# pratyushkumar211/industrial_nnmpc_2021

Measured on AMD Instinct MI355X. Metric: condensed-QP solves/sec (CDU offline datagen), higher is better.
Workload: dtype f64; 1 GPU; cdu_offline_data: synthetic CDU-size plant (n=4480 vars, m=8960 box rows, n_aug=284), 100000 sampled x0 per GPU per step, whole sequences u* written out; batch_per_gpu=100000, total_batch=100000, method=auto, parallelism=dp1 (sharded samples, 1 RCCL gather of the first moves pe...

## Files before the change

industrial_nnmpc_2021_amd/csrc/qp_predict.h:

```cpp
#pragma once
#include "qp_asm.h"

namespace nnmpc {

typedef __bf16 pbf16x8 __attribute__((ext_vector_type(8)));
typedef float pf32x4 __attribute__((ext_vector_type(4)));
typedef unsigned int pu32x4 __attribute__((ext_vector_type(4)));
typedef unsigned int pu32x2 __attribute__((ext_vector_type(2)));
typedef float pf32x2 __attribute__((ext_vector_type(2)));
typedef __bf16 pbf16x2 __attribute__((ext_vector_type(2)));
typedef _Float16 pf16x2 __attribute__((ext_vector_type(2)));

constexpr int PRED_NW = 8;
constexpr int PRED_MAXIT = 64;
template <int NT> struct PredCfg {
  static constexpr int W = 16 * NT * PRED_NW;
  static constexpr int KS = W / 32;
  static constexpr int LDY = W + 8;
};
constexpr int PRED_W = PredCfg<4>::W;
constexpr int PRED_W2 = PredCfg<8>::W;

struct PredArgs {
  const pu32x4* Hf;
  int iters;
  int* itsum;
  int fac10;
  int adaptive;
  float beta[PRED_MAXIT];
};

template <int NT, int PT> __host__ __device__ constexpr int pred_lds_bytes(int nu) {
  return 16 * PT * PredCfg<NT>::LDY * 2 + 2 * 16 * PT * (nu + 4) * 4 + 16;
}

template <int NT> __host__ __device__ constexpr size_t pred_frag_index(int jtg, int ks, int lane) {
  return (((size_t)(jtg / NT) * PredCfg<NT>::KS + ks) * NT + (jtg % NT)) * 64 + lane;
}

__device__ __forceinline__ unsigned pred_bf16(float x) {
  const unsigned u = __float_as_uint(x);
  return (u + 0x7fffu + ((u >> 16) & 1u)) >> 16;
}

template <int NT, int PT, bool NU4 = true>
__global__ __launch_bounds__(64 * PRED_NW, 2) void asm_predict_k(AsmDev d, PredArgs a) {
  extern __shared__ __attribute__((aligned(16))) unsigned char sm_raw[];
  constexpr int KS = PredCfg<NT>::KS, LDY = PredCfg<NT>::LDY, MR = 16 * PT;
  unsigned short* Y = reinterpret_cast<unsigned short*>(sm_raw);
  const int ldb = d.nu + 4;
  float* lbs = reinterpret_cast<float*>(Y + MR * LDY);
  float* ubs = lbs + MR * ldb;
  int* nviol = reinterpret_cast<int*>(ubs + MR * ldb);
  float* rsum = reinterpret_cast<float*>(nviol + 1);
  constexpr int NTH = 64 * PRED_NW;
  const int tid = threadIdx.x, lane = tid & 63, w = __builtin_amdgcn_readfirstlane(tid >> 6);
  const int li = lane & 15, lq = lane >> 4;
  const int p0 = blockIdx.x * MR;
  for (int i = tid; i < MR * d.nu; i += NTH) {
    const int r = i / d.nu, k = i - r * d.nu;
    const size_t p = (size_t)min(p0 + r, d.nseg - 1);
    lbs[r * ldb + k] = (float)d.lb[p * d.nu + k];
    ubs[r * ldb + k] = (float)d.ub[p * d.nu + k];
  }
  for (int i = tid; i < MR * LDY / 2; i += NTH) reinterpret_cast<unsigned*>(Y)[i] = 0u;
  if (tid == 0) { *nviol = 0; rsum[0] = 0.f; rsum[1] = 0.f; }
  unsigned sx[NT][PT][2], sm[NT][PT][2];
#pragma unroll
  for (int jt = 0; jt < NT; ++jt)
#pragma unroll
    for (int pt = 0; pt < PT; ++pt) {
      const size_t p = (size_t)min(p0 + 16 * pt + li, d.nseg - 1);
      const double* xr = d.xunc + p * d.np + 16 * (w * NT + jt) + 4 * lq;
#pragma unroll
      for (int h = 0; h < 2; ++h) {
        const pf32x2 xu = {fminf(fmaxf((float)xr[2 * h], -60000.f), 60000.f), fminf(fmaxf((float)xr[2 * h + 1], -60000.f), 60000.f)};
        sx[jt][pt][h] = __builtin_bit_cast(unsigned, __builtin_convertvector(xu, pf16x2));
        sm[jt][pt][h] = 0u;
      }
    }
  int kc0[NT];
#pragma unroll
  for (int jt = 0; jt < NT; ++jt) kc0[jt] = (16 * (w * NT + jt) + 4 * lq) % d.nu;
  const bool st_words = (d.n & 3) == 0;
  const bool per32 = 32 % d.nu == 0;
  __syncthreads();
  const __amdgpu_buffer_rsrc_t rH = __builtin_amdgcn_make_buffer_rsrc(const_cast<pu32x4*>(a.Hf), 0, PRED_NW * KS * NT * 1024, 0x00020000);
  const int l16 = lane * 16;
  const int hw0 = w * (KS * NT * 1024);
  auto hload = [&](int ksn, int jt) __attribute__((always_inline)) {
    return __builtin_bit_cast(pu32x4, __builtin_amdgcn_raw_buffer_load_b128(rH, l16 + jt * 1024, hw0 + ksn * (NT * 1024), 0));
  };
  int nit = a.iters;
  int kb = 0;
  for (int it = 0; it < nit; ++it) {
    if (tid == 0) rsum[it & 1] = 0.f;
    pf32x4 acc[NT][PT];
#pragma unroll
    for (int jt = 0; jt < NT; ++jt)
#pragma unroll
      for (int pt = 0; pt < PT; ++pt) acc[jt][pt] = pf32x4{0.f, 0.f, 0.f, 0.f};
#ifdef PRED_NO_MFMA
    if (false) {
#else
    if (it > 0) {
#endif
      constexpr int RD = 3;
      pu32x4 hb[RD][NT];
      asm_sfor<0, RD - 1>([&](auto bc) __attribute__((always_inline)) {
        constexpr int b = decltype(bc)::value;
#pragma unroll
        for (int jt = 0; jt < NT; ++jt) hb[b][jt] = hload(b, jt);
      });
      asm_sfor<0, KS>([&](auto kc) __attribute__((always_inline)) {
        constexpr int ks = decltype(kc)::value, b = ks % RD;
        if constexpr (ks + RD - 1 < KS) {
#pragma unroll
          for (int jt = 0; jt < NT; ++jt) hb[(ks + RD - 1) % RD][jt] = hload(ks + RD - 1, jt);
        }
        pu32x4 yf[PT];
#pragma unroll
        for (int pt = 0; pt < PT; ++pt) yf[pt] = *reinterpret_cast<const pu32x4*>(Y + (16 * pt + li) * LDY + 32 * ks + 8 * lq);
#pragma unroll
        for (int jt = 0; jt < NT; ++jt)
#pragma unroll
          for (int pt = 0; pt < PT; ++pt)
            acc[jt][pt] = __builtin_amdgcn_mfma_f32_16x16x32_bf16(__builtin_bit_cast(pbf16x8, hb[b][jt]), __builtin_bit_cast(pbf16x8, yf[pt]),
                                                                  acc[jt][pt], 0, 0, 0);
        __builtin_amdgcn_sched_barrier(0);
      });
    }
    __syncthreads();
    if (it > 0) kb = rsum[(it - 1) & 1] > 0.f ? 0 : kb + 1;
    const pf32x2 beta2 = {a.beta[kb], a.beta[kb]};
    pf32x2 rdot = {0.f, 0.f};
    int yo = li * LDY + 16 * NT * w + 4 * lq, bo = li * ldb;
    asm volatile("" : "+v"(yo), "+v"(bo));
    unsigned short* Yl = Y + yo;
    const float* lbl = lbs + bo;
    const float* ubl = ubs + bo;
    int nv0 = 0;
#pragma unroll
    for (int pt = 0; pt < PT; ++pt) {
      pf32x4 lb4[2], ub4[2];
#pragma unroll
      for (int jt = 0; jt < NT; ++jt) {
        if constexpr (NU4) {
          if (jt < 2 || !per32) {
            lb4[jt & 1] = *reinterpret_cast<const pf32x4*>(lbl + 16 * pt * ldb + kc0[jt]);
            ub4[jt & 1] = *reinterpret_cast<const pf32x4*>(ubl + 16 * pt * ldb + kc0[jt]);
          }
        } else {
#pragma unroll
          for (int r = 0; r < 4; ++r) {
            const int k = kc0[jt] + r, kk = k >= d.nu ? k - d.nu : k;
            lb4[jt & 1][r] = lbl[16 * pt * ldb + kk];
            ub4[jt & 1][r] = ubl[16 * pt * ldb + kk];
          }
        }
        unsigned short* yp = Yl + 16 * pt * LDY + 16 * jt;
        const pu32x2 yw = *reinterpret_cast<const pu32x2*>(yp);
        unsigned yb[2];
#pragma unroll
        for (int h = 0; h < 2; ++h) {
          const pf32x2 xu = __builtin_convertvector(__builtin_bit_cast(pf16x2, sx[jt][pt][h]), pf32x2);
          const unsigned mw = sm[jt][pt][h], ywd = yw[h];
          const pf32x2 nu = {__uint_as_float(mw << 16), __uint_as_float(mw & 0xffff0000u)};
          const pf32x2 y = {__uint_as_float(ywd << 16), __uint_as_float(ywd & 0xffff0000u)};
          const pf32x2 ac = {acc[jt][pt][2 * h], acc[jt][pt][2 * h + 1]};
#ifdef PRED_NO_EPI
          const pf32x2 wv = xu - ac;
#else
          const pf32x2 wv = y + (xu - ac);
#endif
          const pf32x2 cl = {__builtin_amdgcn_fmed3f(wv[0], lb4[jt & 1][2 * h], ub4[jt & 1][2 * h]),
                             __builtin_amdgcn_fmed3f(wv[1], lb4[jt & 1][2 * h + 1], ub4[jt & 1][2 * h + 1])};
          const pf32x2 nun = wv - cl;
          const pf32x2 dn = nun - nu;
          const pf32x2 yn = beta2 * dn + nun;
          rdot += (y - nun) * dn;
          yb[h] = __builtin_bit_cast(unsigned, __builtin_convertvector(yn, pbf16x2));
          sm[jt][pt][h] = __builtin_bit_cast(unsigned, __builtin_convertvector(nun, pbf16x2));
        }
        *reinterpret_cast<pu32x2*>(yp) = pu32x2{yb[0], yb[1]};
      }
      __builtin_amdgcn_sched_barrier(0);
    }
    {
      float rd = rdot[0] + rdot[1];
      for (int off = 32; off > 0; off >>= 1) rd += __shfl_xor(rd, off);
      if (lane == 0) atomicAdd(&rsum[it & 1], rd);
    }
    if (it == 0 && a.adaptive) {
#pragma unroll
      for (int jt = 0; jt < NT; ++jt)
#pragma unroll
        for (int pt = 0; pt < PT; ++pt)
#pragma unroll
          for (int h = 0; h < 2; ++h) nv0 += ((sm[jt][pt][h] & 0x7fffu) != 0u) + ((sm[jt][pt][h] & 0x7fff0000u) != 0u);
      for (int off = 32; off > 0; off >>= 1) nv0 += __shfl_xor(nv0, off);
      if (lane == 0 && nv0) atomicAdd(nviol, nv0);
    }
    __syncthreads();
    if (it == 0 && a.adaptive) nit = min(a.iters, max(8, (a.fac10 * *nviol) / (10 * MR)));
    if (it == 0 && tid == 0 && a.itsum) atomicAdd(a.itsum, nit - 1);
  }
#pragma unroll
  for (int jt = 0; jt < NT; ++jt) {
    const int c0 = 16 * (w * NT + jt) + 4 * lq;
#pragma unroll
    for (int pt = 0; pt < PT; ++pt) {
      const int p = p0 + 16 * pt + li;
      unsigned wd = 0;
#pragma unroll
      for (int r = 0; r < 4; ++r) {
        const unsigned hb16 = (sm[jt][pt][r >> 1] >> (16 * (r & 1))) & 0xffffu;
        wd |= ((hb16 & 0x7fffu) == 0u ? 0u : ((hb16 >> 15) ? 2u : 1u)) << (8 * r);
      }
      if (p < d.nseg && st_words && c0 + 3 < d.n) *reinterpret_cast<unsigned*>(d.st + (size_t)p * d.n + c0) = wd;
      else if (p < d.nseg) {
#pragma unroll
        for (int r = 0; r < 4; ++r) if (c0 + r < d.n) d.st[(size_t)p * d.n + c0 + r] = (unsigned char)((wd >> (8 * r)) & 0xff);
      }
    }
  }
}

__global__ __launch_bounds__(256) void asm_extent_k(AsmDev d, int c0, int c1, int* cnt) {
  __shared__ int wsum[4];
  const int lane = threadIdx.x & 63, wave = threadIdx.x >> 6;
  int hit = 0;
  for (int q = 0; q < 16; ++q) {
    const int p = blockIdx.x * 64 + wave * 16 + q;
    if (p >= d.nseg) break;
    int v = 0;
    for (int r = c0 + lane; r < c1; r += 64) {
      const int k = r % d.nu;
      const double x = d.xunc[(size_t)p * d.np + r];
      v |= x > d.ub[(size_t)p * d.nu + k] || x < d.lb[(size_t)p * d.nu + k];
    }
    hit += __any(v) ? 1 : 0;
  }
  if (lane == 0) wsum[wave] = hit;
  __syncthreads();
  if (threadIdx.x == 0) { const int t = wsum[0] + wsum[1] + wsum[2] + wsum[3]; if (t) atomicAdd(cnt, t); }
}

}
```

Measured before the change: 8.198 million solves/s.

## Overlap prox epilogue of one column half with MFMA k-steps of the other

Splits each wave's column tiles into two halves across the matrix and reorders the Hessian fragment layout so the K loop runs in quarters. While one half's matvec runs on the MFMA units, the projection and momentum epilogue of the other half is interleaved into the same k-steps, hiding the VALU work behind matrix ops. To free registers, half of the unconstrained-solution values move from registers to LDS. The cost is a more complex software pipeline, extra LDS use, and a changed Y read order that depends on the Y halves being updated in the right sequence.

```diff
diff --git a/industrial_nnmpc_2021_amd/csrc/qp_predict.h b/industrial_nnmpc_2021_amd/csrc/qp_predict.h
--- a/industrial_nnmpc_2021_amd/csrc/qp_predict.h
+++ b/industrial_nnmpc_2021_amd/csrc/qp_predict.h
@@ -31,11 +31,17 @@
 };
 
 template <int NT, int PT> __host__ __device__ constexpr int pred_lds_bytes(int nu) {
-  return 16 * PT * PredCfg<NT>::LDY * 2 + 2 * 16 * PT * (nu + 4) * 4 + 16;
+  return 16 * PT * PredCfg<NT>::LDY * 2 + 2 * 16 * PT * (nu + 4) * 4 + 16 + 16 * PT * PredCfg<NT>::W;
+}
+
+template <int NT> __host__ __device__ constexpr int pred_col_tile(int w, int jt) {
+  return (jt / (NT / 2)) * (PRED_NW * (NT / 2)) + w * (NT / 2) + jt % (NT / 2);
 }
 
 template <int NT> __host__ __device__ constexpr size_t pred_frag_index(int jtg, int ks, int lane) {
-  return (((size_t)(jtg / NT) * PredCfg<NT>::KS + ks) * NT + (jtg % NT)) * 64 + lane;
+  constexpr int NH = NT / 2, KQ = PredCfg<NT>::KS / 2;
+  const int c = jtg / (PRED_NW * NH), w = (jtg / NH) % PRED_NW, j = jtg % NH, h = ks / KQ, kl = ks % KQ;
+  return (((((size_t)w * 2 + h) * 2 + c) * KQ + kl) * NH + j) * 64 + lane;
 }
 
 __device__ __forceinline__ unsigned pred_bf16(float x) {
@@ -53,6 +59,7 @@
   float* ubs = lbs + MR * ldb;
   int* nviol = reinterpret_cast<int*>(ubs + MR * ldb);
   float* rsum = reinterpret_cast<float*>(nviol + 1);
+  pu32x2* xul = reinterpret_cast<pu32x2*>(nviol + 4);
   constexpr int NTH = 64 * PRED_NW;
   const int tid = threadIdx.x, lane = tid & 63, w = __builtin_amdgcn_readfirstlane(tid >> 6);
   const int li = lane & 15, lq = lane >> 4;
@@ -65,149 +72,216 @@
   }
   for (int i = tid; i < MR * LDY / 2; i += NTH) reinterpret_cast<unsigned*>(Y)[i] = 0u;
   if (tid == 0) { *nviol = 0; rsum[0] = 0.f; rsum[1] = 0.f; }
-  unsigned sx[NT][PT][2], sm[NT][PT][2];
+  static_assert(NT % 2 == 0 && (PT == 2 || PT == 4), "the schedule below: NT / 2 tiles per half, 4 / PT k-steps per tile of the prox");
+  constexpr int NH = NT / 2;
+  unsigned sx[NH][PT][2], sm[NT][PT][2];
 #pragma unroll
   for (int jt = 0; jt < NT; ++jt)
 #pragma unroll
     for (int pt = 0; pt < PT; ++pt) {
+      unsigned xp[2];
       const size_t p = (size_t)min(p0 + 16 * pt + li, d.nseg - 1);
-      const double* xr = d.xunc + p * d.np + 16 * (w * NT + jt) + 4 * lq;
+      const double* xr = d.xunc + p * d.np + 16 * pred_col_tile<NT>(w, jt) + 4 * lq;
 #pragma unroll
       for (int h = 0; h < 2; ++h) {
         const pf32x2 xu = {fminf(fmaxf((float)xr[2 * h], -60000.f), 60000.f), fminf(fmaxf((float)xr[2 * h + 1], -60000.f), 60000.f)};
-        sx[jt][pt][h] = __builtin_bit_cast(unsigned, __builtin_convertvector(xu, pf16x2));
+        xp[h] = __builtin_bit_cast(unsigned, __builtin_convertvector(xu, pf16x2));
         sm[jt][pt][h] = 0u;
       }
+      if (jt < NH) { sx[jt % NH][pt][0] = xp[0]; sx[jt % NH][pt][1] = xp[1]; }
+      else xul[((jt - NH) * PT + pt) * NTH + tid] = pu32x2{xp[0], xp[1]};
     }
   int kc0[NT];
 #pragma unroll
-  for (int jt = 0; jt < NT; ++jt) kc0[jt] = (16 * (w * NT + jt) + 4 * lq) % d.nu;
+  for (int jt = 0; jt < NT; ++jt) kc0[jt] = (16 * pred_col_tile<NT>(w, jt) + 4 * lq) % d.nu;
   const bool st_words = (d.n & 3) == 0;
-  const bool per32 = 32 % d.nu == 0;
   __syncthreads();
   const __amdgpu_buffer_rsrc_t rH = __builtin_amdgcn_make_buffer_rsrc(const_cast<pu32x4*>(a.Hf), 0, PRED_NW * KS * NT * 1024, 0x00020000);
   const int l16 = lane * 16;
   const int hw0 = w * (KS * NT * 1024);
-  auto hload = [&](int ksn, int jt) __attribute__((always_inline)) {
-    return __builtin_bit_cast(pu32x4, __builtin_amdgcn_raw_buffer_load_b128(rH, l16 + jt * 1024, hw0 + ksn * (NT * 1024), 0));
+  constexpr int KQ = KS / 2, NS = 4 * KQ;
+  constexpr int RD = 3;
+  constexpr int KPU = 4 / PT;
+  auto hload = [&](int s, int j) __attribute__((always_inline)) {
+    return __builtin_bit_cast(pu32x4, __builtin_amdgcn_raw_buffer_load_b128(rH, l16 + j * 1024, hw0 + s * (NH * 1024), 0));
+  };
+  pu32x4 hb[RD][NH];
+  pu32x4 yf[2][PT];
+  pf32x4 acc[NT][PT];
+  pf32x2 rdot = {0.f, 0.f};
+  pf32x2 beta2 = {a.beta[0], a.beta[0]};
+  int yo, bo, xo;
+  auto launder = [&]() __attribute__((always_inline)) {
+    yo = li * LDY + 16 * NH * w + 4 * lq; bo = li * ldb; xo = tid;
+    asm volatile("" : "+v"(yo), "+v"(bo), "+v"(xo));
+  };
+  auto etile = [&](auto jtc, auto ptc) __attribute__((always_inline)) {
+    constexpr int jt = decltype(jtc)::value, pt = decltype(ptc)::value;
+    const float* lbl = lbs + bo + 16 * pt * ldb;
+    const float* ubl = ubs + bo + 16 * pt * ldb;
+    pf32x4 lb4, ub4;
+    if constexpr (NU4) {
+      lb4 = *reinterpret_cast<const pf32x4*>(lbl + kc0[jt]);
+      ub4 = *reinterpret_cast<const pf32x4*>(ubl + kc0[jt]);
+    } else {
+#pragma unroll
+      for (int r = 0; r < 4; ++r) {
+        const int k = kc0[jt] + r, kk = k >= d.nu ? k - d.nu : k;
+        lb4[r] = lbl[kk];
+        ub4[r] = ubl[kk];
+      }
+    }
+    unsigned short* yp = Y + yo + 16 * pt * LDY + (jt / NH) * (PredCfg<NT>::W / 2) + 16 * (jt % NH);
+    const pu32x2 yw = *reinterpret_cast<const pu32x2*>(yp);
+    unsigned yb[2];
+    unsigned xp[2];
+    if constexpr (jt < NH) {
+      asm volatile("" : "+v"(sx[jt][pt][0]), "+v"(sx[jt][pt][1]));
+      xp[0] = sx[jt][pt][0]; xp[1] = sx[jt][pt][1];
+    } else {
+      const pu32x2 xw = xul[xo + ((jt - NH) * PT + pt) * NTH];
+      xp[0] = xw[0]; xp[1] = xw[1];
+    }
+#pragma unroll
+    for (int h = 0; h < 2; ++h) {
+      const pf32x2 xu = __builtin_convertvector(__builtin_bit_cast(pf16x2, xp[h]), pf32x2);
+      const unsigned mw = sm[jt][pt][h], ywd = yw[h];
+      const pf32x2 nu = {__uint_as_float(mw << 16), __uint_as_float(mw & 0xffff0000u)};
+      const pf32x2 y = {__uint_as_float(ywd << 16), __uint_as_float(ywd & 0xffff0000u)};
+      const pf32x2 ac = {acc[jt][pt][2 * h], acc[jt][pt][2 * h + 1]};
+#ifdef PRED_NO_EPI
+      const pf32x2 wv = xu - ac;
+#else
+      const pf32x2 wv = y + (xu - ac);
+#endif
+      const pf32x2 cl = {__builtin_amdgcn_fmed3f(wv[0], lb4[2 * h], ub4[2 * h]), __builtin_amdgcn_fmed3f(wv[1], lb4[2 * h + 1], ub4[2 * h + 1])};
+      const pf32x2 nun = wv - cl;
+      const pf32x2 dn = nun - nu;
+      const pf32x2 yn = beta2 * dn + nun;
+      rdot += (y - nun) * dn;
+      yb[h] = __builtin_bit_cast(unsigned, __builtin_convertvector(yn, pbf16x2));
+      sm[jt][pt][h] = __builtin_bit_cast(unsigned, __builtin_convertvector(nun, pbf16x2));
+    }
+    *reinterpret_cast<pu32x2*>(yp) = pu32x2{yb[0], yb[1]};
+  };
+  auto ehalf = [&](auto cc) __attribute__((always_inline)) {
+    constexpr int c = decltype(cc)::value;
+    asm_sfor<0, PT>([&](auto ptc) __attribute__((always_inline)) {
+      asm_sfor<0, NH>([&](auto jc) __attribute__((always_inline)) { etile(asm_ic<c * NH + decltype(jc)::value>{}, ptc); });
+      __builtin_amdgcn_sched_barrier(0);
+    });
+  };
+  auto rflush = [&](int slot) __attribute__((always_inline)) {
+    float rd = rdot[0] + rdot[1];
+    for (int off = 32; off > 0; off >>= 1) rd += __shfl_xor(rd, off);
+    if (lane == 0) atomicAdd(&rsum[slot], rd);
+    rdot = pf32x2{0.f, 0.f};
+  };
+  auto kstep = [&](auto sc) __attribute__((always_inline)) {
+#ifndef PRED_NO_MFMA
+    constexpr int s = decltype(sc)::value, c = (s / KQ) & 1, sn = s + RD - 1;
+    if constexpr (sn < NS) {
+#pragma unroll
+      for (int j = 0; j < NH; ++j) hb[sn % RD][j] = hload(sn, j);
+    }
+    auto yread = [&](auto tc) __attribute__((always_inline)) {
+      constexpr int t = decltype(tc)::value, ks = (t / (2 * KQ)) * KQ + t % KQ;
+#pragma unroll
+      for (int pt = 0; pt < PT; ++pt) yf[t & 1][pt] = *reinterpret_cast<const pu32x4*>(Y + (16 * pt + li) * LDY + 32 * ks + 8 * lq);
+    };
+    if constexpr (s % (2 * KQ) == 0) yread(asm_ic<s>{});
+    if constexpr ((s + 1) % (2 * KQ) != 0) yread(asm_ic<s + 1>{});
+#pragma unroll
+    for (int j = 0; j < NH; ++j)
+#pragma unroll
+      for (int pt = 0; pt < PT; ++pt)
+        acc[c * NH + j][pt] = __builtin_amdgcn_mfma_f32_16x16x32_bf16(__builtin_bit_cast(pbf16x8, hb[s % RD][j]), __builtin_bit_cast(pbf16x8, yf[s & 1][pt]),
+                                                                      acc[c * NH + j][pt], 0, 0, 0);
+#endif
+  };
+  auto ringfill = [&]() __attribute__((always_inline)) {
+#ifndef PRED_NO_MFMA
+    asm_sfor<0, RD - 1>([&](auto bc) __attribute__((always_inline)) {
+      constexpr int b = decltype(bc)::value;
+#pragma unroll
+      for (int j = 0; j < NH; ++j) hb[b][j] = hload(b, j);
+    });
+#endif
+  };
+  auto quarter = [&](auto qc, auto ec) __attribute__((always_inline)) {
+    constexpr int q = decltype(qc)::value, c = q & 1;
+    constexpr bool WITH_E = decltype(ec)::value != 0;
+    if constexpr (q < 2) {
+#pragma unroll
+      for (int j = 0; j < NH; ++j)
+#pragma unroll
+        for (int pt = 0; pt < PT; ++pt) acc[c * NH + j][pt] = pf32x4{0.f, 0.f, 0.f, 0.f};
+    }
+    asm_sfor<0, KQ>([&](auto klc) __attribute__((always_inline)) {
+      constexpr int kl = decltype(klc)::value;
+      kstep(asm_ic<q * KQ + kl>{});
+      if constexpr (WITH_E) {
+        if constexpr (kl % KPU == 0) {
+          constexpr int u = kl / KPU;
+          etile(asm_ic<(1 - c) * NH + u % NH>{}, asm_ic<u / NH>{});
+        }
+        if constexpr (kl % KPU == KPU - 1) __builtin_amdgcn_sched_barrier(0);
+      } else {
+        __builtin_amdgcn_sched_barrier(0);
+      }
+    });
   };
   int nit = a.iters;
   int kb = 0;
-  for (int it = 0; it < nit; ++it) {
-    if (tid == 0) rsum[it & 1] = 0.f;
-    pf32x4 acc[NT][PT];
+  launder();
+  ringfill();
+#pragma unroll
+  for (int jt = 0; jt < NT; ++jt)
+#pragma unroll
+    for (int pt = 0; pt < PT; ++pt) acc[jt][pt] = pf32x4{0.f, 0.f, 0.f, 0.f};
+  ehalf(asm_ic<0>{});
+  ehalf(asm_ic<1>{});
+  rflush(0);
+  if (a.adaptive) {
+    int nv0 = 0;
 #pragma unroll
     for (int jt = 0; jt < NT; ++jt)
 #pragma unroll
-      for (int pt = 0; pt < PT; ++pt) acc[jt][pt] = pf32x4{0.f, 0.f, 0.f, 0.f};
-#ifdef PRED_NO_MFMA
-    if (false) {
-#else
-    if (it > 0) {
-#endif
-      constexpr int RD = 3;
-      pu32x4 hb[RD][NT];
-      asm_sfor<0, RD - 1>([&](auto bc) __attribute__((always_inline)) {
-        constexpr int b = decltype(bc)::value;
-#pragma unroll
-        for (int jt = 0; jt < NT; ++jt) hb[b][jt] = hload(b, jt);
-      });
-      asm_sfor<0, KS>([&](auto kc) __attribute__((always_inline)) {
-        constexpr int ks = decltype(kc)::value, b = ks % RD;
-        if constexpr (ks + RD - 1 < KS) {
-#pragma unroll
-          for (int jt = 0; jt < NT; ++jt) hb[(ks + RD - 1) % RD][jt] = hload(ks + RD - 1, jt);
-        }
-        pu32x4 yf[PT];
-#pragma unroll
-        for (int pt = 0; pt < PT; ++pt) yf[pt] = *reinterpret_cast<const pu32x4*>(Y + (16 * pt + li) * LDY + 32 * ks + 8 * lq);
-#pragma unroll
-        for (int jt = 0; jt < NT; ++jt)
-#pragma unroll
-          for (int pt = 0; pt < PT; ++pt)
-            acc[jt][pt] = __builtin_amdgcn_mfma_f32_16x16x32_bf16(__builtin_bit_cast(pbf16x8, hb[b][jt]), __builtin_bit_cast(pbf16x8, yf[pt]),
-                                                                  acc[jt][pt], 0, 0, 0);
-        __builtin_amdgcn_sched_barrier(0);
-      });
-    }
+      for (int pt = 0; pt < PT; ++pt)
+#pragma unroll
+        for (int h = 0; h < 2; ++h) nv0 += ((sm[jt][pt][h] & 0x7fffu) != 0u) + ((sm[jt][pt][h] & 0x7fff0000u) != 0u);
+    for (int off = 32; off > 0; off >>= 1) nv0 += __shfl_xor(nv0, off);
+    if (lane == 0 && nv0) atomicAdd(nviol, nv0);
+  }
+  __syncthreads();
+  if (a.adaptive) nit = min(a.iters, max(8, (a.fac10 * *nviol) / (10 * MR)));
+  if (tid == 0 && a.itsum) atomicAdd(a.itsum, nit - 1);
+  if (nit > 1) {
+    quarter(asm_ic<0>{}, asm_ic<0>{});
+    quarter(asm_ic<1>{}, asm_ic<0>{});
     __syncthreads();
-    if (it > 0) kb = rsum[(it - 1) & 1] > 0.f ? 0 : kb + 1;
-    const pf32x2 beta2 = {a.beta[kb], a.beta[kb]};
-    pf32x2 rdot = {0.f, 0.f};
-    int yo = li * LDY + 16 * NT * w + 4 * lq, bo = li * ldb;
-    asm volatile("" : "+v"(yo), "+v"(bo));
-    unsigned short* Yl = Y + yo;
-    const float* lbl = lbs + bo;
-    const float* ubl = ubs + bo;
-    int nv0 = 0;
-#pragma unroll
-    for (int pt = 0; pt < PT; ++pt) {
-      pf32x4 lb4[2], ub4[2];
-#pragma unroll
-      for (int jt = 0; jt < NT; ++jt) {
-        if constexpr (NU4) {
-          if (jt < 2 || !per32) {
-            lb4[jt & 1] = *reinterpret_cast<const pf32x4*>(lbl + 16 * pt * ldb + kc0[jt]);
-            ub4[jt & 1] = *reinterpret_cast<const pf32x4*>(ubl + 16 * pt * ldb + kc0[jt]);
-          }
-        } else {
-#pragma unroll
-          for (int r = 0; r < 4; ++r) {
-            const int k = kc0[jt] + r, kk = k >= d.nu ? k - d.nu : k;
-            lb4[jt & 1][r] = lbl[16 * pt * ldb + kk];
-            ub4[jt & 1][r] = ubl[16 * pt * ldb + kk];
-          }
-        }
-        unsigned short* yp = Yl + 16 * pt * LDY + 16 * jt;
-        const pu32x2 yw = *reinterpret_cast<const pu32x2*>(yp);
-        unsigned yb[2];
-#pragma unroll
-        for (int h = 0; h < 2; ++h) {
-          const pf32x2 xu = __builtin_convertvector(__builtin_bit_cast(pf16x2, sx[jt][pt][h]), pf32x2);
-          const unsigned mw = sm[jt][pt][h], ywd = yw[h];
-          const pf32x2 nu = {__uint_as_float(mw << 16), __uint_as_float(mw & 0xffff0000u)};
-          const pf32x2 y = {__uint_as_float(ywd << 16), __uint_as_float(ywd & 0xffff0000u)};
-          const pf32x2 ac = {acc[jt][pt][2 * h], acc[jt][pt][2 * h + 1]};
-#ifdef PRED_NO_EPI
-          const pf32x2 wv = xu - ac;
-#else
-          const pf32x2 wv = y + (xu - ac);
-#endif
-          const pf32x2 cl = {__builtin_amdgcn_fmed3f(wv[0], lb4[jt & 1][2 * h], ub4[jt & 1][2 * h]),
-                             __builtin_amdgcn_fmed3f(wv[1], lb4[jt & 1][2 * h + 1], ub4[jt & 1][2 * h + 1])};
-          const pf32x2 nun = wv - cl;
-          const pf32x2 dn = nun - nu;
-          const pf32x2 yn = beta2 * dn + nun;
-          rdot += (y - nun) * dn;
-          yb[h] = __builtin_bit_cast(unsigned, __builtin_convertvector(yn, pbf16x2));
-          sm[jt][pt][h] = __builtin_bit_cast(unsigned, __builtin_convertvector(nun, pbf16x2));
-        }
-        *reinterpret_cast<pu32x2*>(yp) = pu32x2{yb[0], yb[1]};
-      }
-      __builtin_amdgcn_sched_barrier(0);
-    }
-    {
-      float rd = rdot[0] + rdot[1];
-      for (int off = 32; off > 0; off >>= 1) rd += __shfl_xor(rd, off);
-      if (lane == 0) atomicAdd(&rsum[it & 1], rd);
-    }
-    if (it == 0 && a.adaptive) {
-#pragma unroll
-      for (int jt = 0; jt < NT; ++jt)
-#pragma unroll
-        for (int pt = 0; pt < PT; ++pt)
-#pragma unroll
-          for (int h = 0; h < 2; ++h) nv0 += ((sm[jt][pt][h] & 0x7fffu) != 0u) + ((sm[jt][pt][h] & 0x7fff0000u) != 0u);
-      for (int off = 32; off > 0; off >>= 1) nv0 += __shfl_xor(nv0, off);
-      if (lane == 0 && nv0) atomicAdd(nviol, nv0);
-    }
-    __syncthreads();
-    if (it == 0 && a.adaptive) nit = min(a.iters, max(8, (a.fac10 * *nviol) / (10 * MR)));
-    if (it == 0 && tid == 0 && a.itsum) atomicAdd(a.itsum, nit - 1);
+    for (int it = 1;; ++it) {
+      kb = rsum[(it - 1) & 1] > 0.f ? 0 : kb + 1;
+      beta2 = pf32x2{a.beta[kb], a.beta[kb]};
+      launder();
+      quarter(asm_ic<2>{}, asm_ic<0>{});
+      quarter(asm_ic<3>{}, asm_ic<1>{});
+      ringfill();
+      __syncthreads();
+      if (it + 1 >= nit) break;
+      if (tid == 0) rsum[(it + 1) & 1] = 0.f;
+      launder();
+      quarter(asm_ic<0>{}, asm_ic<1>{});
+      rflush(it & 1);
+      quarter(asm_ic<1>{}, asm_ic<0>{});
+      __syncthreads();
+    }
+    launder();
+    ehalf(asm_ic<1>{});
   }
 #pragma unroll
   for (int jt = 0; jt < NT; ++jt) {
-    const int c0 = 16 * (w * NT + jt) + 4 * lq;
+    const int c0 = 16 * pred_col_tile<NT>(w, jt) + 4 * lq;
 #pragma unroll
     for (int pt = 0; pt < PT; ++pt) {
       const int p = p0 + 16 * pt + li;
```

Result: faster. 8.300 million solves/s, median of 6 (+1.2%).
